# maxrossi91/moni-align

Hardware: AMD Instinct MI355X
Metric: aligned reads/s (whole node), 150 bp SE, mouse-chr19-scale x12-haplotype index (higher is better)
Workload: dtype u64/int32

## Files before the change

include/moni_hip.h:

```cpp
#ifndef MONI_HIP_H
#define MONI_HIP_H

#include <stddef.h>
#include <stdint.h>

#ifdef __cplusplus
extern "C" {
#endif

#define MONI_OK 0
#define MONI_EINVAL (-22)
#define MONI_ENOMEM (-12)
#define MONI_EIO (-5)
#define MONI_ENODEV (-19)
#define MONI_ERANGE (-34)

typedef struct moni_index moni_index_t;
typedef struct moni_ctx moni_ctx_t;

typedef struct {
    uint64_t n;
    uint64_t r;
    uint64_t w;
    uint64_t n_seq;
// ... 418 lines not shown
int moni_ldx_rewrite(const char *in_path, const char *out_path, int with_w);
int moni_ldx_write(const moni_flat_index_t *idx, const char *path, int with_w);
int moni_ldx_lift_batch(const char *path, int device, const uint64_t *pos, uint64_t n, uint64_t *out);

int moni_ms_file_info(const char *path, uint64_t *n, uint64_t *r);
int moni_ms_file_read(const char *path, uint64_t r, uint64_t *F, uint8_t *heads, uint64_t *starts, uint64_t *ssa, uint64_t *esa,
                      uint64_t *thr, uint64_t *slcp, char *err, uint64_t err_cap);
int moni_ms_file_write(const moni_flat_index_t *idx, const char *path);
int moni_index_load_reference(const char *ms_path, const char *ldx_path, const char *text_path, int device, moni_index_t **out);

int moni_last_kernel_ms(moni_ctx_t *ctx, int which, float *ms);
int moni_last_counters(moni_ctx_t *ctx, uint64_t out[4]);
int moni_seed_occ_stats(moni_ctx_t *ctx, uint64_t out[6]);
int moni_seed_prefilter(moni_ctx_t *ctx, int mode);
int moni_seed_prefilter_stats(moni_ctx_t *ctx, uint64_t out[4]);
const char *moni_version(void);

#ifdef __cplusplus
}
#endif
#endif
```

moni_align_amd/capi.py:

```python
from __future__ import annotations

import ctypes as C
import os
import subprocess
from typing import Dict, Optional

import numpy as np

os.environ.setdefault("GPU_MAX_HW_QUEUES", "16")

HERE = os.path.dirname(os.path.abspath(__file__))
CSRC = os.path.join(HERE, "csrc")
LIB_PATH = os.environ.get("MONI_HIP_LIB") or os.path.join(CSRC, "libmoni_hip.so")

EXPORTS = [
    "moni_version", "moni_index_create", "moni_index_load", "moni_index_destroy", "moni_index_n", "moni_index_r",
    "moni_index_device_bytes", "moni_index_text", "moni_ctx_create", "moni_ctx_destroy", "moni_reads_upload", "moni_reads_swap", "moni_ms_run",
    "moni_ms_query_batch", "moni_seed_run", "moni_seed_counts", "moni_seed_fetch", "moni_seed_batch", "moni_free",
    "moni_phi_lcp_batch", "moni_extz_batch", "moni_last_kernel_ms", "moni_last_counters", "moni_seed_occ_stats",
    "moni_seed_prefilter", "moni_seed_prefilter_stats",
    "moni_align_params_default", "moni_align_batch", "moni_align_csv_batch", "moni_align_run", "moni_align_stream", "moni_sam_header",
    "moni_ldx_info", "moni_ldx_rewrite", "moni_ldx_lift_batch", "moni_ldx_write",
    "moni_ms_file_info", "moni_ms_file_read", "moni_ms_file_write", "moni_index_load_reference", "moni_ms_lengths_batch", "moni_report_mems_batch",
    "moni_pe_params_default", "moni_pe_learn_batch", "moni_pe_align_batch", "moni_pe_align_stream", "moni_pe_align_run", "moni_pe_align_csv_batch", "moni_pe_report_mems_batch",
    "moni_extend_params_default", "moni_extend_batch", "moni_extend_run",
    "moni_pml_batch", "moni_pml_run", "moni_pml_fetch", "moni_pml_sizes",
    "moni_screen_params_default", "moni_screen_run", "moni_screen_sizes", "moni_screen_fetch", "moni_screen_batch",
    "moni_locate_params_default", "moni_locate_run", "moni_locate_sizes", "moni_locate_fetch", "moni_locate_batch",
    "moni_seqcount_params_default", "moni_seqcount_run", "moni_seqcount_sizes", "moni_seqcount_fetch", "moni_seqcount_batch",
    "moni_loci_params_default", "moni_loci_run", "moni_loci_sizes", "moni_loci_fetch", "moni_loci_batch",
    "moni_approx_params_default", "moni_approx_run", "moni_approx_sizes", "moni_approx_fetch", "moni_approx_batch",
    "moni_mslong_params_default", "moni_ms_long_batch",
    "moni_bgzf_params_default", "moni_bgzf_compress",
    "moni_bam_params_default", "moni_bam_set_header", "moni_bam_records",
    "moni_bam_sorted_run", "moni_bam_sort", "moni_bam_merge_plan", "moni_bam_plan_free",
# ... 391 lines not shown
                                      C.POINTER(C.c_void_p), C.POINTER(C.c_void_p), C.POINTER(C.c_uint64)]
        L.moni_approx_params_default.argtypes = [C.POINTER(ApproxParamsC)]
        L.moni_approx_params_default.restype = None
        L.moni_approx_run.argtypes = [C.c_void_p, C.POINTER(ApproxParamsC)]
        L.moni_approx_sizes.argtypes = [C.c_void_p, C.POINTER(C.c_uint64), C.POINTER(C.c_uint64), C.POINTER(C.c_uint64)]
        L.moni_approx_fetch.argtypes = [C.c_void_p] + [C.c_void_p] * 5
        L.moni_approx_batch.argtypes = [C.c_void_p, C.POINTER(ReadBatchC), C.POINTER(ApproxParamsC), C.c_void_p] + [C.POINTER(C.c_void_p)] * 4 + [C.POINTER(C.c_uint64)] * 2
        L.moni_locate_batch.argtypes = [C.c_void_p, C.POINTER(ReadBatchC), C.POINTER(LocateParamsC), C.c_void_p, C.POINTER(C.c_void_p), C.POINTER(C.c_void_p),
                                        C.POINTER(C.c_void_p), C.POINTER(C.c_uint64)]
        L.moni_sam_header.argtypes = [C.c_void_p, C.POINTER(C.c_void_p), C.POINTER(C.c_uint64)]
        L.moni_last_kernel_ms.argtypes = [C.c_void_p, C.c_int, C.POINTER(C.c_float)]
        L.moni_last_counters.argtypes = [C.c_void_p, C.c_void_p]
        L.moni_seed_occ_stats.argtypes = [C.c_void_p, C.c_void_p]
        L.moni_seed_prefilter.argtypes = [C.c_void_p, C.c_int]
        L.moni_seed_prefilter_stats.argtypes = [C.c_void_p, C.c_void_p]
        L.moni_ms_lengths_batch.argtypes = [C.c_void_p, C.POINTER(ReadBatchC), C.c_void_p, C.c_void_p]
        L.moni_mslong_params_default.argtypes = [C.POINTER(MslongParamsC)]
        L.moni_mslong_params_default.restype = None
        L.moni_ms_long_batch.argtypes = [C.c_void_p, C.POINTER(ReadBatchC), C.POINTER(MslongParamsC), C.c_void_p, C.c_void_p, C.POINTER(MslongStatsC)]
        L.moni_report_mems_batch.argtypes = [C.c_void_p, C.POINTER(ReadBatchC), C.c_void_p, C.c_void_p, C.c_void_p, C.POINTER(AlignParamsC),
                                             C.POINTER(C.c_void_p), C.POINTER(C.c_uint64)]
        L.moni_ldx_info.argtypes = [C.c_char_p, C.POINTER(C.c_uint64), C.POINTER(C.c_uint64), C.POINTER(C.c_uint64), C.POINTER(C.c_int)]
        L.moni_ldx_rewrite.argtypes = [C.c_char_p, C.c_char_p, C.c_int]
        L.moni_ldx_write.argtypes = [C.POINTER(FlatIndexC), C.c_char_p, C.c_int]
        L.moni_ms_file_info.argtypes = [C.c_char_p, C.POINTER(C.c_uint64), C.POINTER(C.c_uint64)]
        L.moni_ms_file_read.argtypes = [C.c_char_p, C.c_uint64] + [C.c_void_p] * 7 + [C.c_char_p, C.c_uint64]
        L.moni_ms_file_write.argtypes = [C.POINTER(FlatIndexC), C.c_char_p]
        L.moni_index_load_reference.argtypes = [C.c_char_p, C.c_char_p, C.c_char_p, C.c_int, C.POINTER(C.c_void_p)]
        L.moni_ldx_lift_batch.argtypes = [C.c_char_p, C.c_int, C.c_void_p, C.c_uint64, C.c_void_p]
        L.moni_bgzf_params_default.argtypes = [C.POINTER(BgzfParamsC)]
# ... 153 lines not shown
        self._L = lib()
        self._h = C.c_void_p()
        self._keep = fi
        if reference is not None:
            ms, ldx, text = reference
            _chk(self._L.moni_index_load_reference(ms.encode(), ldx.encode(), text.encode() if text else None, device, C.byref(self._h)), "moni_index_load_reference")
        elif fi is not None:
            st = flat_struct(fi, without_text, without_lcp)
            _chk(self._L.moni_index_create(C.byref(st), device, C.byref(self._h)), "moni_index_create")
        else:
            _chk(self._L.moni_index_load(path.encode(), device, C.byref(self._h)), "moni_index_load")
        self.n = self._L.moni_index_n(self._h)
        self.r = self._L.moni_index_r(self._h)
        self.device_bytes = self._L.moni_index_device_bytes(self._h)

    def text(self) -> np.ndarray:
        out = np.empty(self.n - 1, dtype=np.uint8)
        _chk(self._L.moni_index_text(self._h, out.ctypes.data, out.size), "moni_index_text")
        return out

    def close(self):
        if self._h:
            self._L.moni_index_destroy(self._h)
            self._h = C.c_void_p()


class Ctx:
    def __init__(self, index: Index):
        self._L = lib()
        self.index = index
# ... 684 lines not shown

    def seed_occ_stats(self) -> Dict[str, int]:
        out = np.zeros(6, dtype=np.uint64)
        _chk(self._L.moni_seed_occ_stats(self._h, out.ctypes.data), "moni_seed_occ_stats")
        return dict(zip(("long_seeds", "overflow_used", "overflow_cap", "count_passes", "long_launches", "compactions"), (int(v) for v in out)))

    def seed_prefilter(self, mode: int) -> None:
        _chk(self._L.moni_seed_prefilter(self._h, int(mode)), "moni_seed_prefilter")

    def seed_prefilter_stats(self) -> Dict[str, float]:
        out = np.zeros(4, dtype=np.uint64)
        _chk(self._L.moni_seed_prefilter_stats(self._h, out.ctypes.data), "moni_seed_prefilter_stats")
        return {"tasks": int(out[0]), "skipped": int(out[1]), "lookups": int(out[2]), "density": float(out[3]) / 1e6}


def ldx_info(path: str):
    n_seq, u, w, has_w = C.c_uint64(), C.c_uint64(), C.c_uint64(), C.c_int()
    _chk(lib().moni_ldx_info(path.encode(), C.byref(n_seq), C.byref(u), C.byref(w), C.byref(has_w)), "moni_ldx_info")
    return {"n_seq": n_seq.value, "u": u.value, "w": w.value, "has_w": bool(has_w.value)}


def ldx_rewrite(src: str, dst: str, with_w: bool):
    _chk(lib().moni_ldx_rewrite(src.encode(), dst.encode(), int(with_w)), "moni_ldx_rewrite")


def ldx_write(fi, path: str, with_w: bool = True):
    st = flat_struct(fi)
    _chk(lib().moni_ldx_write(C.byref(st), path.encode(), int(with_w)), "moni_ldx_write")


# ... 29 lines not shown
```

moni_align_amd/csrc/moni_hip.hip:

```cpp
#include <hip/hip_runtime.h>
#include <fcntl.h>
#include <sys/mman.h>
#include <sys/stat.h>
#include <unistd.h>
#include <cstring>
#include <atomic>
#include <chrono>
#include <rocprim/device/device_scan.hpp>
#include <rocprim/device/device_radix_sort.hpp>
#include <rocprim/iterator/transform_iterator.hpp>

#include <sched.h>
#include <cstdio>
#include <cstdlib>
#include <cstring>
#include <string>
#include <thread>
#include <algorithm>
#include <vector>

#include "../../include/moni_hip.h"
#include "owned_buf.hpp"
#include "image.hpp"
#include "lift_build.hpp"
// ... 61 lines not shown
using Stream = Handle<hipStream_t, hipStreamDestroy>;
using Event = Handle<hipEvent_t, hipEventDestroy>;

struct moni_index {
    int device = 0;
    moni_consts_t K;
    DBuf<moni_tables_t> d_tables;
    DBuf<moni_row_t> d_rows;
    DBuf<moni_frow_t> d_frows;
    DBuf<uint32_t> d_cr;
    DBuf<moni_rec_t> d_recs;
    DBuf<moni_phi_t> d_phi, d_phi_inv;
    DBuf<uint32_t> d_phi_dir, d_phi_inv_dir;
    DBuf<uint8_t> d_text;
    DBuf<uint64_t> d_text2; DBuf<uint32_t> d_exc; uint32_t exc_sh = 10, exc_words = 0;
    DBuf<uint32_t> d_kmers; uint32_t pf_k = 0; double pf_density = 0; bool pf_on = false; float pf_build_ms = 0; bool compl_acgt = false;
    DBuf<uint64_t> d_seq_starts;
    DBuf<uint32_t> d_name_id;
    DBuf<uint8_t> d_snames; DBuf<uint32_t> d_sname_off;
    DBuf<moni_lift_seq_t> d_lift_seqs; DBuf<moni_lift_run_t> d_lift_runs;
    DBuf<uint64_t> d_pdir;
    bool lifts_null = true;
    uint64_t bytes = 0;
    std::vector<uint8_t> h_text;
    mh::HostIndex hix;
};

#define PE_NSET 1
#define PE_NSTREAM 4
#ifndef AK_NSET
// ... 11 lines not shown
    DBuf<moni_locate_res_t> res; DBuf<uint64_t> toe, cnt, off;
    int ensure(uint64_t n_tasks) { int rc; return (rc = res.ensure(n_tasks + 1)) || (rc = toe.ensure(n_tasks + 1)) || (rc = cnt.ensure(n_tasks + 2)) || (rc = off.ensure(n_tasks + 2)) ? rc : MONI_OK; }
};
struct moni_ctx : ResidentBatch {
    moni_index* idx = nullptr;
    Stream stream;
    Event ev[EV_N];
    bool ev_valid[EV_N] = {};
    std::vector<ResidentBatch> stash;
    DBuf<uint64_t> ptr, pat; DBuf<uint8_t> pflag;
    DBuf<uint32_t> cnt_m, cnt_s;
    DBuf<uint64_t> pf_flag, pf_pos, pf_live; DBuf<unsigned long long> pf_stats;
    int seed_prefilter = 1;
    bool seed_fuse = true;
    DBuf<uint64_t> evl; DBuf<uint32_t> evl_cnt;
    bool ms_events = true;
    bool pf_active = false;
    uint64_t pf_tasks = 0;
    DBuf<moni_u64x2> mem_slots;
    DBuf<uint64_t> tot, read_mem_off;
    DBuf<moni_mem_t> mems;
    DBuf<uint32_t> aux;
    DBuf<uint64_t> lowers, tmp;
    DBuf<uint64_t> long_list;
    DBuf<uint64_t> occ_cnt, occ_off, occs;
    DBuf<moni_mem_t> mems_compact;
    bool occs_valid = false;
    uint64_t ovf_cap = 4096;
    uint64_t occ_stats[6] = {0, 0, 0, 0, 0, 0};
    DBuf<uint32_t> pool;
// ... 308 lines not shown
        (rc = upload(I->d_text, text, I->bytes)) || (rc = upload(I->d_seq_starts, img.seq_starts, I->bytes)) ||
        (rc = upload(I->d_name_id, name_id, I->bytes)) || (rc = upload(I->d_snames, sname_blob, I->bytes)) || (rc = upload(I->d_sname_off, sname_off, I->bytes))) {
        moni_index_destroy(I);
        return rc;
    }
    {
        const uint64_t n_text = f->n - 1, n_words = n_text / 32 + 2;
        I->exc_sh = text2_exc_shift(n_text, MONI_EXC_BITS);
        I->exc_words = (uint32_t)((((n_text >> I->exc_sh) + 1) + 31) / 32);
        if (I->d_text2.alloc_exact(n_words) || I->d_exc.alloc_exact((size_t)I->exc_words + 1)) { moni_index_destroy(I); return MONI_ENOMEM; }
        I->bytes += n_words * 8 + (uint64_t)I->exc_words * 4;
        if (hipMemset(I->d_exc.p, 0, (size_t)I->exc_words * 4 + 4) != hipSuccess) { moni_index_destroy(I); return MONI_ENODEV; }
        hipLaunchKernelGGL(text2_build_kernel, dim3((unsigned)((n_words + 255) / 256)), dim3(256), 0, 0, I->d_text.p, n_text, n_words, I->d_text2.p, I->d_exc.p, I->exc_sh);
        if (hipGetLastError() != hipSuccess || hipDeviceSynchronize() != hipSuccess) { moni_index_destroy(I); return MONI_ENODEV; }
    }
    {
        const uint64_t n_text = f->n - 1, n_words = n_text / 32 + 1;
        I->pf_k = pf_choose_k(n_text);
        if (const char* v = getenv("MONI_PREFILTER_K")) { const int x = atoi(v); if (x >= (int)PF_K_MIN && x <= (int)PF_K_MAX) I->pf_k = (uint32_t)x; }
        const uint64_t tw = pf_table_words(I->pf_k);
        DBuf<unsigned long long> d_pop;
        Event e0, e1;
        if (I->d_kmers.alloc_exact(tw) || d_pop.alloc_exact(1)) { moni_index_destroy(I); return MONI_ENOMEM; }
        I->bytes += tw * 4;
        if (hipEventCreate(&e0.h) != hipSuccess || hipEventCreate(&e1.h) != hipSuccess || hipEventRecord(e0, 0) != hipSuccess ||
            hipMemsetAsync(I->d_kmers.p, 0, tw * 4, 0) != hipSuccess || hipMemsetAsync(d_pop.p, 0, 8, 0) != hipSuccess) { moni_index_destroy(I); return MONI_ENODEV; }
        hipLaunchKernelGGL(kmer_build_kernel, dim3((unsigned)((n_words + 255) / 256)), dim3(256), 0, 0, I->d_text.p, n_text, n_words, I->pf_k, I->d_kmers.p);
        hipLaunchKernelGGL(kmer_popcount_kernel, dim3((unsigned)std::min<uint64_t>((tw + 255) / 256, 4096)), dim3(256), 0, 0, I->d_kmers.p, tw, d_pop.p);
        unsigned long long pop = 0;
        if (hipEventRecord(e1, 0) != hipSuccess || hipGetLastError() != hipSuccess || hipMemcpy(&pop, d_pop.p, 8, hipMemcpyDeviceToHost) != hipSuccess ||
// ... 101 lines not shown
int moni_index_text(const moni_index_t* I, uint8_t* out, uint64_t cap) {
    if (!I || !out || cap < I->h_text.size()) return MONI_EINVAL;
    memcpy(out, I->h_text.data(), I->h_text.size());
    return MONI_OK;
}

int moni_ctx_create(moni_index_t* I, moni_ctx_t** out) {
    if (!I || !out) return MONI_EINVAL;
    HIPCHK(hipSetDevice(I->device));
    moni_ctx* c = new moni_ctx();
    c->idx = I;
    if (const char* v = getenv("MONI_MS_VARIANT")) c->ms_variant = atoi(v);
    if (const char* v = getenv("MONI_EXTZ_LDS")) c->extz_lds = atoi(v);
    if (const char* v = getenv("MONI_SEED_FUSE")) c->seed_fuse = atoi(v) != 0;
    if (const char* v = getenv("MONI_MS_EVENTS")) c->ms_events = atoi(v) != 0;
    if (const char* v = getenv("MONI_SEED_PREFILTER")) { const int x = atoi(v); if (x >= 0 && x <= 2) c->seed_prefilter = x; }
    bool ok = hipStreamCreate(&c->stream.h) == hipSuccess;
    for (int i = 0; ok && i < EV_N; ++i) ok = hipEventCreate(&c->ev[i].h) == hipSuccess;
    ok = ok && c->d_small.alloc_exact(1) == MONI_OK && c->d_counters.alloc_exact(4) == MONI_OK && c->pf_stats.alloc_exact(2) == MONI_OK &&
         hipMemset(c->pf_stats.p, 0, 2 * sizeof(unsigned long long)) == hipSuccess && hipMemset(c->d_small.p, 0, sizeof(occ_small_t)) == hipSuccess && hipMemset(c->d_counters.p, 0, 4 * sizeof(unsigned long long)) == hipSuccess;
    if (!ok) { fprintf(stderr, "moni_hip: context creation failed on device %d\n", I->device); moni_ctx_destroy(c); return MONI_ENODEV; }
    *out = c;
    return MONI_OK;
}

void moni_ctx_destroy(moni_ctx_t* c) {
    if (!c) return;
    (void)hipSetDevice(c->idx->device);
    if (c->stream) (void)hipStreamSynchronize(c->stream);
    delete c;
}

static void results_invalidate(moni_ctx* c) {
    c->n_mems = c->n_occs = 0; c->occs_valid = false; c->pml.valid = false; c->scr.valid = false; c->loc.valid = false; c->sc.valid = false; c->apx.valid = false; c->loci.valid = false;
}

static int reads_upload(moni_ctx* c, const moni_read_batch_t* b, bool keep_host_copy);
int moni_reads_upload(moni_ctx_t* c, const moni_read_batch_t* b) { return reads_upload(c, b, true); }

static int reads_upload(moni_ctx* c, const moni_read_batch_t* b, bool keep_host_copy) {
    if (!c || !b || !b->offsets || (b->n_reads && !b->seq)) return MONI_EINVAL;
    HIPCHK(hipSetDevice(c->idx->device));
    const uint64_t nr = b->n_reads;
    uint64_t mx = 0;
// ... 70 lines not shown
    const uint64_t* live = nullptr; const uint64_t* n_live = nullptr;
    if (n_tasks && filter_min_len) {
        if ((rc = c->pf_flag.ensure(n_tasks + 2)) || (rc = c->pf_pos.ensure(n_tasks + 2)) || (rc = c->pf_live.ensure(n_tasks + 2))) return rc;
        if (!fuse)
            hipLaunchKernelGGL(strand_filter_kernel, dim3((unsigned)((n_tasks + 1 + MS_BLOCK - 1) / MS_BLOCK)), dim3(MS_BLOCK), 0, c->stream, c->pat.p, c->offs.p, c->blk.p, c->pflag.p, n_tasks,
                               filter_min_len, I->pf_k, I->d_kmers.p, c->pf_flag.p, c->cnt_m.p, c->cnt_s.p, c->pf_stats.p);
        if ((rc = exclusive_scan_u64(c, c->pf_flag.p, c->pf_pos.p, n_tasks + 1))) return rc;
        hipLaunchKernelGGL(live_list_kernel, dim3((unsigned)((n_tasks + 255) / 256)), dim3(256), 0, c->stream, c->pf_flag.p, c->pf_pos.p, n_tasks, c->pf_live.p);
        live = c->pf_live.p; n_live = c->pf_pos.p + n_tasks;
        c->pf_active = true;
    }
    if (n_tasks && events) {
#define MS_LAUNCH(NCH, MINW, STAGED) do { const uint64_t nl = (n_tasks + (NCH) - 1) / (NCH); \
        hipLaunchKernelGGL((ms_lf_events_kernel<NCH, MINW, STAGED>), dim3((unsigned)((nl + MS_BLOCK - 1) / MS_BLOCK)), dim3(MS_BLOCK), 0, c->stream, \
                           I->K, tabs, I->d_rows.p, I->d_frows.p, I->d_cr.p, I->d_recs.p, c->pat.p, c->offs.p, c->blk.p, n_tasks, c->evl.p, c->evl_cnt.p, c->d_counters.p, live, n_live); } while (0)
        switch (c->ms_variant) {
            case 1: MS_LAUNCH(1, 8, MONI_MS_EV_STAGE != 0); break;
            case 2: MS_LAUNCH(2, 8, false); break;
            case 3: MS_LAUNCH(2, 6, false); break;
            case 4: MS_LAUNCH(1, 6, MONI_MS_EV_STAGE != 0); break;
            case 5: MS_LAUNCH(4, 4, false); break;
            default: MS_LAUNCH(1, 6, MONI_MS_EV_STAGE != 0); break;
        }
#undef MS_LAUNCH
    } else if (n_tasks) {
#define MS_LAUNCH(NCH, MINW) do { const uint64_t nl = (n_tasks + (NCH) - 1) / (NCH); \
        hipLaunchKernelGGL((ms_lf_kernel<NCH, MINW>), dim3((unsigned)((nl + MS_BLOCK - 1) / MS_BLOCK)), dim3(MS_BLOCK), 0, c->stream, \
                           I->K, tabs, I->d_rows.p, I->d_frows.p, I->d_cr.p, I->d_recs.p, c->pat.p, c->offs.p, c->blk.p, n_tasks, c->ptr.p, c->d_counters.p, live, n_live); } while (0)
        switch (c->ms_variant) {
            case 1: MS_LAUNCH(1, 8); break;
// ... 72 lines not shown

static int seed_all(moni_ctx* c, const moni_seed_params_t* prm, bool align_path) {
    moni_index* I = c->idx;
    const uint64_t nr = c->n_reads, n_tasks = 2 * nr;
    int rc;
    if ((rc = c->cnt_m.ensure(n_tasks + 2)) || (rc = c->cnt_s.ensure(n_tasks + 2)) || (rc = c->tot.ensure(nr + 2)) ||
        (rc = c->read_mem_off.ensure(nr + 2)) || (rc = c->mem_slots.ensure(n_tasks * MONI_MEM_SLOTS + 1)))
        return rc;
    uint32_t* cnt_m = c->cnt_m.p; uint32_t* cnt_s = c->cnt_s.p;
    uint64_t* tot = c->tot.p; uint64_t* rmo = c->read_mem_off.p;
    moni_u64x2* slots = c->mem_slots.p;
    const uint64_t* offs = c->offs.p;
    HIPCHK(hipMemsetAsync(c->d_counters.p, 0, 4 * sizeof(unsigned long long), c->stream));
    HIPCHK(hipMemsetAsync(c->d_small.p, 0, sizeof(occ_small_t), c->stream));
    HIPCHK(hipMemsetAsync(c->pf_stats.p, 0, 2 * sizeof(unsigned long long), c->stream));
    c->pf_tasks = n_tasks;
    const bool filter = (c->seed_prefilter == 2 || (c->seed_prefilter == 1 && align_path)) && I->pf_on && prm->min_len >= I->pf_k;
    rec(c, EV_ALL0);
    const bool events = c->ms_events && c->max_len < MONI_EV_MAX_LEN;
    if ((rc = ms_launch(c, nullptr, filter ? prm->min_len : 0, events))) return rc;
    const uint64_t* live = c->pf_active ? c->pf_live.p : nullptr; const uint64_t* n_live = c->pf_active ? c->pf_pos.p + n_tasks : nullptr;
    const uint64_t* pat = c->pat.p; const uint64_t* ptr = events ? nullptr : c->ptr.p;
    const uint64_t* ev = c->evl.p; const uint32_t* ev_cnt = c->evl_cnt.p;
    const unsigned grid_t = (unsigned)((n_tasks + MS_BLOCK - 1) / MS_BLOCK);
    const uint32_t split_on = prm->report_mems ? 0u : 1u;
    static const bool mem_bytes = getenv("MONI_MEM_BYTES") != nullptr;
    const uint64_t* text2 = mem_bytes ? nullptr : I->d_text2.p;
#define MEM_LAUNCH(EMIT, RMO, MEMS, AUX, LIVE, NLIVE) do { \
        if (events && c->max_len <= 160) hipLaunchKernelGGL((mem_events_kernel<EMIT, 5>), dim3(grid_t), dim3(MS_BLOCK), 0, c->stream, I->K, I->d_text.p, text2, I->d_exc.p, I->exc_sh, I->exc_words, pat, offs, c->blk.p, \
                                                  n_tasks, ev, ev_cnt, prm->min_len, split_on, cnt_m, cnt_s, RMO, MEMS, AUX, slots, c->d_counters.p, LIVE, NLIVE); \
// ... 102 lines not shown
    return seed_all(c, prm, true);
}

int moni_seed_prefilter(moni_ctx_t* c, int mode) {
    if (!c || mode < 0 || mode > 2) return MONI_EINVAL;
    c->seed_prefilter = mode;
    return MONI_OK;
}

int moni_seed_prefilter_stats(moni_ctx_t* c, uint64_t out[4]) {
    if (!c || !out) return MONI_EINVAL;
    HIPCHK(hipSetDevice(c->idx->device));
    unsigned long long h[2];
    HIPCHK(hipMemcpy(h, c->pf_stats.p, sizeof(h), hipMemcpyDeviceToHost));
    out[0] = c->pf_tasks; out[1] = h[0]; out[2] = h[1]; out[3] = (uint64_t)(c->idx->pf_density * 1e6 + 0.5);
    return MONI_OK;
}

int moni_seed_counts(moni_ctx_t* c, uint64_t* n_mems, uint64_t* n_occs) {
    if (!c) return MONI_EINVAL;
    if (n_mems) *n_mems = c->n_mems;
    if (n_occs) *n_occs = c->n_occs;
    return MONI_OK;
}

int moni_seed_fetch(moni_ctx_t* c, moni_mem_t* mems, uint64_t* occs, uint64_t* read_mem_off) {
    if (!c) return MONI_EINVAL;
    HIPCHK(hipSetDevice(c->idx->device));
    if ((mems || occs) && c->n_mems) {
        int rc = seed_compact(c);
// ... 1045 lines not shown
```

moni_align_amd/csrc/seed_core.h:

```cpp
#pragma once
#include <stdint.h>

#include "../../include/moni_hip.h"
#include "layout.h"

#if defined(__HIPCC__)
#define MONI_HD __host__ __device__ __forceinline__
#else
#define MONI_HD inline
#endif

#if defined(__HIP_DEVICE_COMPILE__)
#define MONI_ATOMIC_INC_U32(p) atomicAdd((p), 1u)
#define MONI_FLAG_SET(p) atomicExch((p), 1u)
#else
#define MONI_ATOMIC_INC_U32(p) ((*(p))++)
#define MONI_FLAG_SET(p) (*(p) = 1u)
#endif

#define MONI_MEM_SLOTS 4u
struct alignas(16) moni_u64x2 { uint64_t x, y; };
struct alignas(32) moni_u64x4 { uint64_t x, y, z, w; };

struct lds_tables_t {
// ... 195 lines not shown
    S.abs = true;
}

#if defined(MONI_MS_ATTR) && MONI_MS_ATTR == 1
#define MS_ATTR_WALK(nj) ((nj) += (1ull << 28))
#define MS_ATTR_GEN(nj)
#elif defined(MONI_MS_ATTR) && MONI_MS_ATTR == 2
#define MS_ATTR_WALK(nj)
#define MS_ATTR_GEN(nj) ((nj) += (1ull << 28))
#else
#define MS_ATTR_WALK(nj)
#define MS_ATTR_GEN(nj)
#endif
MONI_HD void ms_step(const moni_consts_t& K, const lds_tables_t& L, const moni_row_t* __restrict__ rows,
                     const moni_frow_t* __restrict__ frows, const uint32_t* __restrict__ cr, const moni_rec_t* __restrict__ recs,
                     uint32_t c, ms_state_t& S, unsigned long long& n_jumps) {
    if (S.abs) {
        moni_row_t A;
        settle_run(rows, K.r, S.pos, S.run, A);
        S.off = (uint32_t)(S.pos - row_start(A));
        if (S.pos - row_start(A) >= MONI_ROW_LEN_SAT) { MS_ATTR_GEN(n_jumps); ms_step_general(K, L, rows, cr, recs, c, S, n_jumps); return; }
        S.abs = false;
    }
    const uint32_t hc = L.hot_slot[c];
    while (true) {
        const moni_frow_t* __restrict__ fr = frows + S.run;
        const moni_u64x2 q0 = *reinterpret_cast<const moni_u64x2*>(&fr->w[0]);
        const uint64_t w0 = q0.x;
        const uint32_t len = (uint32_t)w0 & 0xFFFu;
        if (!((w0 >> 58) & 1u) || hc >= 4) {
            const moni_row_t A = ld_row(rows, S.run);
            if (S.off == MONI_OFF_END) S.pos = ld_start(rows, S.run + 1) - 1;
            else S.pos = row_start(A) + S.off;
            MS_ATTR_GEN(n_jumps);
            ms_step_general(K, L, rows, cr, recs, c, S, n_jumps);
            return;
        }
        if (S.off == MONI_OFF_END) S.off = len - 1;
        if (S.off >= len) { S.off -= len; ++S.run; MS_ATTR_WALK(n_jumps); continue; }
        const uint32_t hh = (uint32_t)(w0 >> 56) & 3u;
        if (hc == hh) {
            S.sample--;
// ... 148 lines not shown
                            moni_u64x2 two; two.x = stage[(uint64_t)i * stage_stride]; two.y = stage[(uint64_t)(i + 1u) * stage_stride];
                            *reinterpret_cast<moni_u64x2*>(ev + eb[k] + (ne[k] - j) + i) = two;
                        }
                    }
                } else ev[eb[k] + ne[k]] = w;
                ++ne[k];
            }
            if (s + 1u == S[k].m) {
                if (STAGED) {
                    const uint32_t rem = ne[k] & (MONI_EV_STAGE_N - 1u);
                    for (uint32_t i = 0; i < rem; ++i) ev[eb[k] + (ne[k] - rem) + i] = stage[(uint64_t)i * stage_stride];
                }
                ev_cnt[tk[k]] = ne[k];
            }
        }
    }
}

struct mem_src_dense_t {
    static constexpr bool skips = false;
    const uint64_t* p = nullptr; uint64_t nxt = 0;
    MONI_HD void open(const uint64_t* __restrict__ ptr, const moni_u64x2* __restrict__ blk, uint64_t task, uint32_t m) {
        p = ptr + ws_ptr_base(blk, task);
        nxt = m ? p[(uint64_t)(m - 1) * 64u] : 0;
    }
    MONI_HD uint64_t take(uint32_t s) { const uint64_t pos = nxt; if (s) nxt = p[(uint64_t)(s - 1u) * 64u]; return pos; }
    MONI_HD uint32_t silent(uint32_t) const { return 0; }
};
template <bool SKIP>
struct mem_src_events_t {
// ... 413 lines not shown
```

moni_align_amd/csrc/seed_kernels.hip:

```cpp
#include <hip/hip_runtime.h>
#include <stdint.h>

#include "seed_core.h"
#include "prefilter_core.h"
#include "packfilter_core.h"

#define MS_BLOCK 256
#ifndef MS_CHAINS
#define MS_CHAINS 2
#endif
#ifndef OCC_STAGE
#define OCC_STAGE 1
#endif

__device__ __forceinline__ void load_tables(lds_tables_t& L, const moni_tables_t* __restrict__ T, const moni_consts_t& K) {
    if (threadIdx.x < MONI_MAX_SIGMA) {
        L.rec_base[threadIdx.x] = K.rec_base[threadIdx.x];
        L.rec_cnt[threadIdx.x] = K.rec_cnt[threadIdx.x];
        L.hot_slot[threadIdx.x] = K.hot_slot[threadIdx.x];
    }
    for (int i = threadIdx.x; i < 256; i += blockDim.x) {
        L.code[i] = T->code[i];
        L.compl_tab[i] = T->compl_tab[i];
        L.c2[i] = base_acgt((uint32_t)i) ? (uint8_t)base2((uint32_t)i) : (uint8_t)4;
// ... 46 lines not shown
                    const uint64_t* __restrict__ live, const uint64_t* __restrict__ n_live) {
    if (live) {
        n_tasks = *n_live;
        if ((uint64_t)blockIdx.x * MS_BLOCK * NCH >= n_tasks) return;
    }
    __shared__ lds_tables_t L;
    __shared__ uint64_t ST[STAGED ? MONI_EV_STAGE_N : 1][STAGED ? MS_BLOCK : 1];
    load_tables(L, T, K);
    const uint64_t task0 = ((uint64_t)blockIdx.x * MS_BLOCK + threadIdx.x) * NCH;
    unsigned long long n_steps = 0, n_jumps = 0;
    if (task0 < n_tasks)
        ms_task_events<NCH, STAGED>(K, L, rows, frows, cr, recs, pat, offs, blk, n_tasks, task0, ev, ev_cnt, n_steps, n_jumps, live,
                                    STAGED ? &ST[0][threadIdx.x] : nullptr, MS_BLOCK);
    wave_add(n_steps, &counters[0]);
    wave_add(n_jumps, &counters[1]);
}

template <bool EMIT, int W, class SRC>
__device__ __forceinline__ void
mem_body(const moni_consts_t& K, const uint8_t* __restrict__ text, const uint64_t* __restrict__ text2, const uint32_t* __restrict__ exc, uint32_t exc_sh, uint32_t exc_words,
           const uint64_t* __restrict__ pat, const uint64_t* __restrict__ offs, const moni_u64x2* __restrict__ blk, uint64_t n_tasks,
           const uint64_t* __restrict__ ptr, uint32_t min_len, uint32_t split_on,
           uint32_t* __restrict__ cnt_m, uint32_t* __restrict__ cnt_s,
           const uint64_t* __restrict__ read_mem_off, moni_mem_t* __restrict__ mems, uint32_t* __restrict__ aux,
           moni_u64x2* __restrict__ slots, unsigned long long* __restrict__ counters,
           const uint64_t* __restrict__ live, const uint64_t* __restrict__ n_live, const SRC& src) {
    if (live) {
        n_tasks = *n_live;
        if ((uint64_t)blockIdx.x * MS_BLOCK >= n_tasks) return;
    }
// ... 213 lines not shown
```

Measured before the change: 44.19 million.

## Leap over matching-statistics LF steps using sampled ISA and text comparison

Adds a sampled inverse suffix array and a per-sample table of clean ACGT run lengths, both built on the GPU when the index loads. A new matching-statistics kernel watches for runs of LF steps that produce no jump. After enough such steps it compares the read directly against the packed text and, when the match is long enough, jumps ahead to the sampled ISA entry instead of stepping base by base. The aim is to cut the serial, latency-bound LF walk for highly repetitive haplotype indexes, in exchange for extra index memory, build time, and a more divergent state machine per thread.

```diff
diff --git a/include/moni_hip.h b/include/moni_hip.h
--- a/include/moni_hip.h
+++ b/include/moni_hip.h
@@ -456,6 +456,8 @@
 int moni_seed_occ_stats(moni_ctx_t *ctx, uint64_t out[6]);
 int moni_seed_prefilter(moni_ctx_t *ctx, int mode);
 int moni_seed_prefilter_stats(moni_ctx_t *ctx, uint64_t out[4]);
+int moni_ms_leap_stats(moni_ctx_t *ctx, uint64_t out[4]);
+int moni_index_leap_table(const moni_index_t *index, uint64_t *isa, uint8_t *clean, uint64_t cap, uint64_t *n_entries, uint32_t *stride, float *build_ms);
 const char *moni_version(void);
 
 #ifdef __cplusplus
diff --git a/moni_align_amd/capi.py b/moni_align_amd/capi.py
--- a/moni_align_amd/capi.py
+++ b/moni_align_amd/capi.py
@@ -18,7 +18,7 @@
     "moni_index_device_bytes", "moni_index_text", "moni_ctx_create", "moni_ctx_destroy", "moni_reads_upload", "moni_reads_swap", "moni_ms_run",
     "moni_ms_query_batch", "moni_seed_run", "moni_seed_counts", "moni_seed_fetch", "moni_seed_batch", "moni_free",
     "moni_phi_lcp_batch", "moni_extz_batch", "moni_last_kernel_ms", "moni_last_counters", "moni_seed_occ_stats",
-    "moni_seed_prefilter", "moni_seed_prefilter_stats",
+    "moni_seed_prefilter", "moni_seed_prefilter_stats", "moni_ms_leap_stats", "moni_index_leap_table",
     "moni_align_params_default", "moni_align_batch", "moni_align_csv_batch", "moni_align_run", "moni_align_stream", "moni_sam_header",
     "moni_ldx_info", "moni_ldx_rewrite", "moni_ldx_lift_batch", "moni_ldx_write",
     "moni_ms_file_info", "moni_ms_file_read", "moni_ms_file_write", "moni_index_load_reference", "moni_ms_lengths_batch", "moni_report_mems_batch",
@@ -440,6 +440,8 @@
         L.moni_seed_occ_stats.argtypes = [C.c_void_p, C.c_void_p]
         L.moni_seed_prefilter.argtypes = [C.c_void_p, C.c_int]
         L.moni_seed_prefilter_stats.argtypes = [C.c_void_p, C.c_void_p]
+        L.moni_ms_leap_stats.argtypes = [C.c_void_p, C.c_void_p]
+        L.moni_index_leap_table.argtypes = [C.c_void_p, C.c_void_p, C.c_void_p, C.c_uint64, C.POINTER(C.c_uint64), C.POINTER(C.c_uint32), C.POINTER(C.c_float)]
         L.moni_ms_lengths_batch.argtypes = [C.c_void_p, C.POINTER(ReadBatchC), C.c_void_p, C.c_void_p]
         L.moni_mslong_params_default.argtypes = [C.POINTER(MslongParamsC)]
         L.moni_mslong_params_default.restype = None
@@ -623,6 +625,15 @@
         self.r = self._L.moni_index_r(self._h)
         self.device_bytes = self._L.moni_index_device_bytes(self._h)
 
+    def leap_table(self, fetch: bool = True):
+        n_ent, stride, ms = C.c_uint64(), C.c_uint32(), C.c_float()
+        _chk(self._L.moni_index_leap_table(self._h, None, None, 0, C.byref(n_ent), C.byref(stride), C.byref(ms)), "moni_index_leap_table")
+        isa = np.zeros(n_ent.value if fetch else 0, dtype=np.uint64)
+        clean = np.zeros(n_ent.value if fetch else 0, dtype=np.uint8)
+        if fetch and n_ent.value:
+            _chk(self._L.moni_index_leap_table(self._h, isa.ctypes.data, clean.ctypes.data, n_ent.value, None, None, None), "moni_index_leap_table")
+        return {"stride": int(stride.value), "build_ms": float(ms.value), "isa": isa, "clean": clean}
+
     def text(self) -> np.ndarray:
         out = np.empty(self.n - 1, dtype=np.uint8)
         _chk(self._L.moni_index_text(self._h, out.ctypes.data, out.size), "moni_index_text")
@@ -1337,6 +1348,12 @@
         return {"tasks": int(out[0]), "skipped": int(out[1]), "lookups": int(out[2]), "density": float(out[3]) / 1e6}
 
 
+    def ms_leap_stats(self) -> Dict[str, int]:
+        out = np.zeros(4, dtype=np.uint64)
+        _chk(self._L.moni_ms_leap_stats(self._h, out.ctypes.data), "moni_ms_leap_stats")
+        return dict(zip(("leaps", "steps_leapt", "comparisons", "stride"), (int(v) for v in out)))
+
+
 def ldx_info(path: str):
     n_seq, u, w, has_w = C.c_uint64(), C.c_uint64(), C.c_uint64(), C.c_int()
     _chk(lib().moni_ldx_info(path.encode(), C.byref(n_seq), C.byref(u), C.byref(w), C.byref(has_w)), "moni_ldx_info")
diff --git a/moni_align_amd/csrc/moni_hip.hip b/moni_align_amd/csrc/moni_hip.hip
--- a/moni_align_amd/csrc/moni_hip.hip
+++ b/moni_align_amd/csrc/moni_hip.hip
@@ -99,6 +99,7 @@
     DBuf<uint32_t> d_phi_dir, d_phi_inv_dir;
     DBuf<uint8_t> d_text;
     DBuf<uint64_t> d_text2; DBuf<uint32_t> d_exc; uint32_t exc_sh = 10, exc_words = 0;
+    DBuf<uint64_t> d_isa, d_clean; uint32_t leap_sh = 0; float leap_build_ms = 0;
     DBuf<uint32_t> d_kmers; uint32_t pf_k = 0; double pf_density = 0; bool pf_on = false; float pf_build_ms = 0; bool compl_acgt = false;
     DBuf<uint64_t> d_seq_starts;
     DBuf<uint32_t> d_name_id;
@@ -140,6 +141,8 @@
     int seed_prefilter = 1;
     bool seed_fuse = true;
     DBuf<uint64_t> evl; DBuf<uint32_t> evl_cnt;
+    bool ms_leap = true;
+    DBuf<unsigned long long> leap_stats;
     bool ms_events = true;
     bool pf_active = false;
     uint64_t pf_tasks = 0;
@@ -478,6 +481,23 @@
         hipLaunchKernelGGL(text2_build_kernel, dim3((unsigned)((n_words + 255) / 256)), dim3(256), 0, 0, I->d_text.p, n_text, n_words, I->d_text2.p, I->d_exc.p, I->exc_sh);
         if (hipGetLastError() != hipSuccess || hipDeviceSynchronize() != hipSuccess) { moni_index_destroy(I); return MONI_ENODEV; }
     }
+    if (const char* v = getenv("MONI_MS_LEAP"); !v || atoi(v) != 0) {
+        const uint64_t n = f->n, r = f->r;
+        uint32_t sh = MONI_LEAP_SH;
+        if (const char* w = getenv("MONI_MS_LEAP_STRIDE")) { const int x = atoi(w); if (x == 8) sh = 3; else if (x == 16) sh = 4; else if (x == 32) sh = 5; }
+        const uint64_t n_ent = ((n - 1) >> sh) + 1, clean_words = n_ent / 8 + 2, chunk = 4096;
+        DBuf<uint64_t> d_ssa;
+        Event e0, e1;
+        if (I->d_isa.alloc_exact(n_ent + 2) || I->d_clean.alloc_exact(clean_words) || d_ssa.alloc_exact(r + 1)) { moni_index_destroy(I); return MONI_ENOMEM; }
+        I->bytes += (n_ent + 2) * 8 + clean_words * 8;
+        if (hipMemcpy(d_ssa.p, f->ssa, r * 8, hipMemcpyHostToDevice) != hipSuccess || hipEventCreate(&e0.h) != hipSuccess || hipEventCreate(&e1.h) != hipSuccess ||
+            hipEventRecord(e0, 0) != hipSuccess || hipMemsetAsync(I->d_isa.p, 0, (n_ent + 2) * 8, 0) != hipSuccess || hipMemsetAsync(I->d_clean.p, 0, clean_words * 8, 0) != hipSuccess) { moni_index_destroy(I); return MONI_ENODEV; }
+        hipLaunchKernelGGL(leap_clean_kernel, dim3((unsigned)(((n + chunk - 1) / chunk + 255) / 256)), dim3(256), 0, 0, I->d_text.p, n - 1, n, chunk, sh, reinterpret_cast<uint8_t*>(I->d_clean.p));
+        hipLaunchKernelGGL(isa_build_kernel, dim3((unsigned)((r + 255) / 256)), dim3(256), 0, 0, I->d_rows.p, r, n, d_ssa.p, sh, I->d_isa.p, reinterpret_cast<uint8_t*>(I->d_clean.p));
+        if (hipEventRecord(e1, 0) != hipSuccess || hipGetLastError() != hipSuccess || hipEventSynchronize(e1) != hipSuccess || hipEventElapsedTime(&I->leap_build_ms, e0, e1) != hipSuccess) { moni_index_destroy(I); return MONI_ENODEV; }
+        I->leap_sh = sh;
+        if (getenv("MONI_AK_PROFILE")) fprintf(stderr, "moni_hip: leap tables: stride %u, %.1f MB, built in %.2f ms\n", 1u << sh, ((n_ent + 2) * 8 + clean_words * 8) / 1e6, I->leap_build_ms);
+    }
     {
         const uint64_t n_text = f->n - 1, n_words = n_text / 32 + 1;
         I->pf_k = pf_choose_k(n_text);
@@ -609,11 +629,12 @@
     if (const char* v = getenv("MONI_EXTZ_LDS")) c->extz_lds = atoi(v);
     if (const char* v = getenv("MONI_SEED_FUSE")) c->seed_fuse = atoi(v) != 0;
     if (const char* v = getenv("MONI_MS_EVENTS")) c->ms_events = atoi(v) != 0;
+    if (const char* v = getenv("MONI_MS_LEAP")) c->ms_leap = atoi(v) != 0;
     if (const char* v = getenv("MONI_SEED_PREFILTER")) { const int x = atoi(v); if (x >= 0 && x <= 2) c->seed_prefilter = x; }
     bool ok = hipStreamCreate(&c->stream.h) == hipSuccess;
     for (int i = 0; ok && i < EV_N; ++i) ok = hipEventCreate(&c->ev[i].h) == hipSuccess;
-    ok = ok && c->d_small.alloc_exact(1) == MONI_OK && c->d_counters.alloc_exact(4) == MONI_OK && c->pf_stats.alloc_exact(2) == MONI_OK &&
-         hipMemset(c->pf_stats.p, 0, 2 * sizeof(unsigned long long)) == hipSuccess && hipMemset(c->d_small.p, 0, sizeof(occ_small_t)) == hipSuccess && hipMemset(c->d_counters.p, 0, 4 * sizeof(unsigned long long)) == hipSuccess;
+    ok = ok && c->d_small.alloc_exact(1) == MONI_OK && c->d_counters.alloc_exact(4) == MONI_OK && c->pf_stats.alloc_exact(2) == MONI_OK && c->leap_stats.alloc_exact(4) == MONI_OK &&
+         hipMemset(c->pf_stats.p, 0, 2 * sizeof(unsigned long long)) == hipSuccess && hipMemset(c->leap_stats.p, 0, 4 * sizeof(unsigned long long)) == hipSuccess && hipMemset(c->d_small.p, 0, sizeof(occ_small_t)) == hipSuccess && hipMemset(c->d_counters.p, 0, 4 * sizeof(unsigned long long)) == hipSuccess;
     if (!ok) { fprintf(stderr, "moni_hip: context creation failed on device %d\n", I->device); moni_ctx_destroy(c); return MONI_ENODEV; }
     *out = c;
     return MONI_OK;
@@ -623,6 +644,13 @@
     if (!c) return;
     (void)hipSetDevice(c->idx->device);
     if (c->stream) (void)hipStreamSynchronize(c->stream);
+    if (getenv("MONI_AK_PROFILE") && c->leap_stats.p && c->pf_stats.p && c->d_counters.p) {
+        unsigned long long lp[4] = {0, 0, 0, 0}, pf[2] = {0, 0}, cn[4] = {0, 0, 0, 0};
+        if (hipMemcpy(lp, c->leap_stats.p, sizeof lp, hipMemcpyDeviceToHost) == hipSuccess && hipMemcpy(pf, c->pf_stats.p, sizeof pf, hipMemcpyDeviceToHost) == hipSuccess &&
+            hipMemcpy(cn, c->d_counters.p, sizeof cn, hipMemcpyDeviceToHost) == hipSuccess)
+            fprintf(stderr, "moni_hip: last seeding run: %llu tasks, %llu skipped by the prefilter, S %llu, J %llu; %llu leaps, %llu steps leapt, %llu comparisons\n",
+                    (unsigned long long)c->pf_tasks, pf[0], cn[0], cn[1], lp[0], lp[1], lp[2]);
+    }
     delete c;
 }
 
@@ -723,6 +751,13 @@
 #define MS_LAUNCH(NCH, MINW, STAGED) do { const uint64_t nl = (n_tasks + (NCH) - 1) / (NCH); \
         hipLaunchKernelGGL((ms_lf_events_kernel<NCH, MINW, STAGED>), dim3((unsigned)((nl + MS_BLOCK - 1) / MS_BLOCK)), dim3(MS_BLOCK), 0, c->stream, \
                            I->K, tabs, I->d_rows.p, I->d_frows.p, I->d_cr.p, I->d_recs.p, c->pat.p, c->offs.p, c->blk.p, n_tasks, c->evl.p, c->evl_cnt.p, c->d_counters.p, live, n_live); } while (0)
+        const bool leap = c->ms_leap && I->d_isa.p && I->d_text2.p && MONI_MS_EV_STAGE != 0 && (c->ms_variant == 0 || c->ms_variant == 4 || c->ms_variant > 5 || c->ms_variant < 0);
+        if (leap) {
+            ms_leap_t Z; Z.isa = I->d_isa.p; Z.clean = I->d_clean.p; Z.text2 = I->d_text2.p; Z.n_text = I->K.n_text; Z.sh = I->leap_sh;
+            hipLaunchKernelGGL((ms_lf_leap_kernel<6>), dim3((unsigned)((n_tasks + MS_BLOCK - 1) / MS_BLOCK)), dim3(MS_BLOCK), 0, c->stream,
+                               I->K, tabs, I->d_rows.p, I->d_frows.p, I->d_cr.p, I->d_recs.p, c->pat.p, c->offs.p, c->blk.p, n_tasks, c->evl.p, c->evl_cnt.p, c->d_counters.p, live, n_live,
+                               Z, c->pflag.p, c->leap_stats.p);
+        } else
         switch (c->ms_variant) {
             case 1: MS_LAUNCH(1, 8, MONI_MS_EV_STAGE != 0); break;
             case 2: MS_LAUNCH(2, 8, false); break;
@@ -825,6 +860,7 @@
     HIPCHK(hipMemsetAsync(c->d_counters.p, 0, 4 * sizeof(unsigned long long), c->stream));
     HIPCHK(hipMemsetAsync(c->d_small.p, 0, sizeof(occ_small_t), c->stream));
     HIPCHK(hipMemsetAsync(c->pf_stats.p, 0, 2 * sizeof(unsigned long long), c->stream));
+    HIPCHK(hipMemsetAsync(c->leap_stats.p, 0, 4 * sizeof(unsigned long long), c->stream));
     c->pf_tasks = n_tasks;
     const bool filter = (c->seed_prefilter == 2 || (c->seed_prefilter == 1 && align_path)) && I->pf_on && prm->min_len >= I->pf_k;
     rec(c, EV_ALL0);
@@ -957,6 +993,29 @@
     unsigned long long h[2];
     HIPCHK(hipMemcpy(h, c->pf_stats.p, sizeof(h), hipMemcpyDeviceToHost));
     out[0] = c->pf_tasks; out[1] = h[0]; out[2] = h[1]; out[3] = (uint64_t)(c->idx->pf_density * 1e6 + 0.5);
+    return MONI_OK;
+}
+
+int moni_ms_leap_stats(moni_ctx_t* c, uint64_t out[4]) {
+    if (!c || !out) return MONI_EINVAL;
+    HIPCHK(hipSetDevice(c->idx->device));
+    unsigned long long h[4];
+    HIPCHK(hipMemcpy(h, c->leap_stats.p, sizeof(h), hipMemcpyDeviceToHost));
+    out[0] = h[0]; out[1] = h[1]; out[2] = h[2]; out[3] = c->idx->d_isa.p ? 1ull << c->idx->leap_sh : 0;
+    return MONI_OK;
+}
+
+int moni_index_leap_table(const moni_index_t* I, uint64_t* isa, uint8_t* clean, uint64_t cap, uint64_t* n_entries, uint32_t* stride, float* build_ms) {
+    if (!I) return MONI_EINVAL;
+    const uint64_t n_ent = I->d_isa.p ? ((I->K.n - 1) >> I->leap_sh) + 1 : 0;
+    if (n_entries) *n_entries = n_ent;
+    if (stride) *stride = I->d_isa.p ? 1u << I->leap_sh : 0;
+    if (build_ms) *build_ms = I->leap_build_ms;
+    if (!isa && !clean) return MONI_OK;
+    if (cap < n_ent) return MONI_EINVAL;
+    HIPCHK(hipSetDevice(I->device));
+    if (isa && n_ent) HIPCHK(hipMemcpy(isa, I->d_isa.p, n_ent * 8, hipMemcpyDeviceToHost));
+    if (clean && n_ent) HIPCHK(hipMemcpy(clean, I->d_clean.p, n_ent, hipMemcpyDeviceToHost));
     return MONI_OK;
 }
 
diff --git a/moni_align_amd/csrc/seed_core.h b/moni_align_amd/csrc/seed_core.h
--- a/moni_align_amd/csrc/seed_core.h
+++ b/moni_align_amd/csrc/seed_core.h
@@ -233,8 +233,9 @@
 #endif
 MONI_HD void ms_step(const moni_consts_t& K, const lds_tables_t& L, const moni_row_t* __restrict__ rows,
                      const moni_frow_t* __restrict__ frows, const uint32_t* __restrict__ cr, const moni_rec_t* __restrict__ recs,
-                     uint32_t c, ms_state_t& S, unsigned long long& n_jumps) {
+                     uint32_t c, ms_state_t& S, unsigned long long& n_jumps, bool have_pre = false, moni_u64x2 pre = moni_u64x2()) {
     if (S.abs) {
+        have_pre = false;
         moni_row_t A;
         settle_run(rows, K.r, S.pos, S.run, A);
         S.off = (uint32_t)(S.pos - row_start(A));
@@ -244,7 +245,8 @@
     const uint32_t hc = L.hot_slot[c];
     while (true) {
         const moni_frow_t* __restrict__ fr = frows + S.run;
-        const moni_u64x2 q0 = *reinterpret_cast<const moni_u64x2*>(&fr->w[0]);
+        const moni_u64x2 q0 = have_pre ? pre : *reinterpret_cast<const moni_u64x2*>(&fr->w[0]);
+        have_pre = false;
         const uint64_t w0 = q0.x;
         const uint32_t len = (uint32_t)w0 & 0xFFFu;
         if (!((w0 >> 58) & 1u) || hc >= 4) {
@@ -423,6 +425,150 @@
                 ev_cnt[tk[k]] = ne[k];
             }
         }
+    }
+}
+
+#define MONI_LEAP_SH 4u
+#ifndef MONI_LEAP_T
+#define MONI_LEAP_T 8u
+#endif
+#ifndef MONI_LEAP_KMIN
+#define MONI_LEAP_KMIN 8u
+#endif
+#define MONI_LEAP_MAX 255u
+struct ms_leap_t {
+    const uint64_t* isa; const uint64_t* clean;
+    const uint64_t* text2;
+    uint64_t n_text; uint32_t sh;
+};
+struct moni_u64pair { uint64_t x, y; };
+
+MONI_HD void isa_walk_run(const moni_row_t* __restrict__ rows, uint64_t r, uint64_t n, uint64_t k, uint64_t ssa_k, uint32_t sh,
+                          uint64_t* __restrict__ isa, uint8_t* __restrict__ clean) {
+    moni_row_t A = ld_row(rows, (uint32_t)k);
+    uint64_t pos = row_lfbase(A), sample = ssa_k % n;
+    uint32_t run = row_dest(A);
+    const uint64_t mask = (1ull << sh) - 1;
+    while (true) {
+        settle_run(rows, r, pos, run, A);
+        const uint64_t off = pos - row_start(A);
+        if (!(sample & mask)) {
+            if (off > 0xFFFFFFFEull) { isa[sample >> sh] = 0; clean[sample >> sh] = 0; }
+            else isa[sample >> sh] = (uint64_t)run | (off << 32);
+        }
+        if (off == 0 || sample == 0) break;
+        pos = row_lfbase(A) + off; run = row_dest(A); --sample;
+    }
+}
+MONI_HD void leap_clean_chunk(const uint8_t* __restrict__ text, uint64_t n_text, uint64_t c0, uint64_t c1, uint32_t sh, uint8_t* __restrict__ clean) {
+    uint32_t cnt = 0;
+    { uint64_t e = c1; while (e < n_text && cnt < MONI_LEAP_MAX && base_acgt(text[e])) { ++e; ++cnt; } }
+    const uint64_t mask = (1ull << sh) - 1;
+    for (uint64_t t = c1; t-- > c0;) {
+        cnt = (t < n_text && base_acgt(text[t])) ? (cnt < MONI_LEAP_MAX ? cnt + 1u : MONI_LEAP_MAX) : 0u;
+        if (!(t & mask)) clean[t >> sh] = (uint8_t)cnt;
+    }
+}
+
+MONI_HD void ms_task_events_leap(const moni_consts_t& K, const lds_tables_t& L, const moni_row_t* __restrict__ rows,
+                                 const moni_frow_t* __restrict__ frows, const uint32_t* __restrict__ cr, const moni_rec_t* __restrict__ recs,
+                                 const uint64_t* __restrict__ pat, const uint64_t* __restrict__ offs, const moni_u64x2* __restrict__ blk, uint64_t n_tasks, uint64_t slot,
+                                 uint64_t* __restrict__ ev, uint32_t* __restrict__ ev_cnt, unsigned long long& n_steps, unsigned long long& n_jumps,
+                                 const uint64_t* __restrict__ live, uint64_t* stage, uint32_t stage_stride,
+                                 const ms_leap_t& Z, const uint8_t* __restrict__ pflag, unsigned long long* stats) {
+    if (slot >= n_tasks) return;
+    const uint64_t task = live ? live[slot] : slot; const uint64_t read = task >> 1;
+    const uint32_t m = (uint32_t)(offs[read + 1] - offs[read]);
+    if (!m) return;
+    const uint64_t pb = ws_pat_base(blk, task), eb = ws_ev_base(blk, task);
+    const uint64_t lb = ws_block_len(blk, task);
+    const uint64_t cb = pb + 64u * ((lb + 7) / 8);
+    const bool has_inv = pflag[task] != 0;
+    const uint32_t stride = 1u << Z.sh;
+    ms_state_t S;
+    S.m = m; S.run = (uint32_t)K.r - 1; S.pos = K.n - 1; S.abs = true; S.off = 0; S.sample = K.last_run_sample; S.word = 0;
+    n_steps += m;
+    enum { STEP = 0, PROBE = 1, ENTRY = 2 };
+    uint32_t mode = STEP, s = 0, ne = 0;
+    uint32_t cnt = 0;
+    uint32_t k = 0;
+    uint64_t t0 = 0;
+    bool capped = false;
+    while (s < m) {
+        const void* pa; const uint64_t* pw;
+        if (mode == STEP) { pa = frows + S.run; pw = pat + pb + (uint64_t)(s >> 3) * 64u; }
+        else if (mode == PROBE) {
+            const uint64_t a = S.sample - 1 - k; const uint32_t qi = m - 1u - s - k, sh = qi & 31u;
+            pa = Z.text2 + ((a >= sh ? a - sh : 0) >> 5); pw = pat + cb + (uint64_t)(qi >> 5) * 64u;
+        } else { pa = Z.isa + (t0 >> Z.sh); pw = Z.clean + (t0 >> (Z.sh + 3u)); }
+        const moni_u64pair qa = *reinterpret_cast<const moni_u64pair*>(pa);
+        const uint64_t qw = *pw;
+        if (mode == STEP) {
+            const uint32_t raw = (uint32_t)(qw >> (8u * (s & 7u))) & 0xFFu;
+            const uint32_t c = L.code[raw];
+            bool assigned = true;
+            if (c == MONI_CODE_ABSENT) {
+                S.sample = 0; S.pos = L.abs_pos[raw]; S.run = L.abs_run[raw]; S.abs = true;
+                cnt = MONI_LEAP_T + 1u;
+            } else {
+                const uint32_t j0 = (uint32_t)n_jumps;
+                moni_u64x2 q0; q0.x = qa.x; q0.y = qa.y;
+                ms_step(K, L, rows, frows, cr, recs, c, S, n_jumps, true, q0);
+                assigned = ((((uint32_t)n_jumps) ^ j0) & 0x0FFFFFFFu) != 0;
+                if (assigned) cnt = 0; else if (cnt <= MONI_LEAP_T) ++cnt;
+            }
+            if (assigned || s == 0) {
+                const uint64_t w = assigned ? (S.sample | ((uint64_t)(s + 1u) << MONI_EV_SHIFT)) : K.last_run_sample;
+                const uint32_t j = ne & (MONI_EV_STAGE_N - 1u);
+                stage[(uint64_t)j * stage_stride] = w;
+                if (j == MONI_EV_STAGE_N - 1u) {
+#pragma unroll
+                    for (uint32_t i = 0; i < MONI_EV_STAGE_N; i += 2) {
+                        moni_u64x2 two; two.x = stage[(uint64_t)i * stage_stride]; two.y = stage[(uint64_t)(i + 1u) * stage_stride];
+                        *reinterpret_cast<moni_u64x2*>(ev + eb + (ne - j) + i) = two;
+                    }
+                }
+                ++ne;
+            }
+            ++s;
+            if (cnt == MONI_LEAP_T && m - s >= stride + MONI_LEAP_KMIN && S.sample - 1 < Z.n_text) { mode = PROBE; k = 0; ++stats[2]; }
+        } else if (mode == PROBE) {
+            const uint64_t a = S.sample - 1 - k; const uint32_t qi = m - 1u - s - k, sh = qi & 31u, ta = (uint32_t)a & 31u;
+            uint32_t lim = sh + 1u;
+            if (a < sh) lim = (uint32_t)a + 1u;
+            uint64_t tw;
+            if ((a >> 5) == ((a >= sh ? a - sh : 0) >> 5)) tw = qa.x << (2u * (31u - ta));
+            else tw = (qa.y << (2u * (31u - ta))) | (qa.x >> (2u * (ta + 1u)));
+            uint64_t x = tw ^ (qw << (2u * (31u - sh)));
+            if (has_inv) x |= pat[cb + 64u * ((lb + 31) / 32) + (uint64_t)(qi >> 5) * 64u] << (2u * (31u - sh));
+            uint32_t eq = x ? (uint32_t)__builtin_clzll(x) >> 1 : 32u;
+            if (eq > lim) eq = lim;
+            k += eq;
+            if (eq < lim || k >= m - s || (uint64_t)k >= S.sample) {
+                mode = STEP; cnt = MONI_LEAP_T + 1u;
+                if (k >= stride + MONI_LEAP_KMIN) {
+                    const uint64_t far = S.sample - k;
+                    t0 = (far + stride - 1u) & ~(uint64_t)(stride - 1u);
+                    capped = S.sample - t0 > MONI_LEAP_MAX;
+                    if (capped) t0 = (S.sample - MONI_LEAP_MAX + stride - 1u) & ~(uint64_t)(stride - 1u);
+                    mode = ENTRY;
+                }
+            }
+        } else {
+            const uint32_t len = (uint32_t)(S.sample - t0);
+            const uint32_t cl = (uint32_t)(qw >> (8u * ((uint32_t)(t0 >> Z.sh) & 7u))) & 0xFFu;
+            mode = STEP;
+            if (cl >= len) {
+                s += len; S.sample = t0; S.run = (uint32_t)qa.x; S.off = (uint32_t)(qa.x >> 32); S.abs = false;
+                ++stats[0]; stats[1] += len;
+                if (capped) cnt = 0;
+            }
+        }
+    }
+    {
+        const uint32_t rem = ne & (MONI_EV_STAGE_N - 1u);
+        for (uint32_t i = 0; i < rem; ++i) ev[eb + (ne - rem) + i] = stage[(uint64_t)i * stage_stride];
+        ev_cnt[task] = ne;
     }
 }
 
diff --git a/moni_align_amd/csrc/seed_kernels.hip b/moni_align_amd/csrc/seed_kernels.hip
--- a/moni_align_amd/csrc/seed_kernels.hip
+++ b/moni_align_amd/csrc/seed_kernels.hip
@@ -84,6 +84,40 @@
                                     STAGED ? &ST[0][threadIdx.x] : nullptr, MS_BLOCK);
     wave_add(n_steps, &counters[0]);
     wave_add(n_jumps, &counters[1]);
+}
+
+template <int MINW>
+__global__ void __launch_bounds__(MS_BLOCK, MINW)
+ms_lf_leap_kernel(const moni_consts_t K, const moni_tables_t* __restrict__ T, const moni_row_t* __restrict__ rows,
+                  const moni_frow_t* __restrict__ frows, const uint32_t* __restrict__ cr, const moni_rec_t* __restrict__ recs,
+                  const uint64_t* __restrict__ pat, const uint64_t* __restrict__ offs, const moni_u64x2* __restrict__ blk, uint64_t n_tasks,
+                  uint64_t* __restrict__ ev, uint32_t* __restrict__ ev_cnt, unsigned long long* __restrict__ counters,
+                  const uint64_t* __restrict__ live, const uint64_t* __restrict__ n_live, const ms_leap_t Z, const uint8_t* __restrict__ pflag,
+                  unsigned long long* __restrict__ leap) {
+    if (live) {
+        n_tasks = *n_live;
+        if ((uint64_t)blockIdx.x * MS_BLOCK >= n_tasks) return;
+    }
+    __shared__ lds_tables_t L;
+    __shared__ uint64_t ST[MONI_EV_STAGE_N][MS_BLOCK];
+    load_tables(L, T, K);
+    const uint64_t slot = (uint64_t)blockIdx.x * MS_BLOCK + threadIdx.x;
+    unsigned long long n_steps = 0, n_jumps = 0, st[3] = {0, 0, 0};
+    ms_task_events_leap(K, L, rows, frows, cr, recs, pat, offs, blk, n_tasks, slot, ev, ev_cnt, n_steps, n_jumps, live, &ST[0][threadIdx.x], MS_BLOCK, Z, pflag, st);
+    wave_add(n_steps, &counters[0]);
+    wave_add(n_jumps, &counters[1]);
+    wave_add(st[0], &leap[0]);
+    wave_add(st[1], &leap[1]);
+    wave_add(st[2], &leap[2]);
+}
+__global__ void __launch_bounds__(256) leap_clean_kernel(const uint8_t* __restrict__ text, uint64_t n_text, uint64_t n, uint64_t chunk, uint32_t sh, uint8_t* __restrict__ clean) {
+    const uint64_t c0 = ((uint64_t)blockIdx.x * 256 + threadIdx.x) * chunk;
+    if (c0 < n) leap_clean_chunk(text, n_text, c0, c0 + chunk < n ? c0 + chunk : n, sh, clean);
+}
+__global__ void __launch_bounds__(256) isa_build_kernel(const moni_row_t* __restrict__ rows, uint64_t r, uint64_t n, const uint64_t* __restrict__ ssa, uint32_t sh,
+                                                        uint64_t* __restrict__ isa, uint8_t* __restrict__ clean) {
+    const uint64_t k = (uint64_t)blockIdx.x * 256 + threadIdx.x;
+    if (k < r) isa_walk_run(rows, r, n, k, ssa[k], sh, isa, clean);
 }
 
 template <bool EMIT, int W, class SRC>
```

New measurement: 45.84 million, median of 6. +3.7%, better.
